# mym-br/gama_tts

Measured on AMD Instinct MI355X. Metric: audio samples/sec (whole node), batched VTM @44.1kHz, higher is better.
Workload: dtype f32

## Files before the change

### gama_tts_amd/capi.py

```python
import ctypes
import os

import numpy as np

_HERE = os.path.dirname(os.path.abspath(__file__))
_LIB_NAME = "libgama_vtm.so"
N_PARAM = 16
DEVICE_NONE = -1
PRECISION_F64 = 0
PRECISION_MIXED = 1
PRECISION_F32 = 2
TUBE_10_6 = 0
TUBE_30_18 = 1
TABLE_FIR, TABLE_SRC_H, TABLE_SRC_DH, TABLE_WAVETABLE = 0, 1, 2, 3
_STATUS_UNSUPPORTED = 4


class GvtmError(RuntimeError):
    def __init__(self, status, message):
        super().__init__("gvtm status %d: %s" % (status, message))
        self.status = status


class Config(ctypes.Structure):
# ... 132 lines not shown
        "gvtm_tracks_frame_count": (sz, [tracks, vp, sz]),
        "gvtm_generate_tracks_device": (i, [i, tracks, vp, vp, sz, sz, vp, vp, vp, vp]),
        "gvtm_synthesize_events_device": (i, [vp, tracks, vp, vp, sz, sz, vp, sz, vp, vp, vp, vp, vp]),
        "gvtm_plan_set_voice_tracks": (i, [vp, tracks, sz]),
        "gvtm_generate_tracks_voices_device": (i, [vp, vp, vp, vp, sz, sz, vp, vp, vp, vp]),
        "gvtm_synthesize_events_voices_device": (i, [vp, vp, vp, vp, sz, sz, vp, sz, vp, vp, vp, vp, vp]),
        "gvtm_tracks_chunks_frame_count": (sz, [tracks, vp, vp, sz]),
        "gvtm_generate_tracks_chunks_device": (i, [vp, vp, vp, vp, vp, sz, sz, vp, vp, vp, vp]),
        "gvtm_synthesize_events_chunks_device": (i, [vp, vp, vp, vp, vp, sz, sz, vp, sz, vp, vp, vp, vp, vp]),
        "gvtm_intonation_apply_host": (i64, [tracks, vp, sz, vp, sz, vp, sz, vp]),
        "gvtm_apply_intonation_device": (i, [vp, vp, vp, sz, vp, vp, vp, vp, sz, vp, sz, vp, vp, vp]),
        "gvtm_synthesize_intonation_device": (i, [vp, vp, vp, sz, vp, vp, vp, vp, sz, sz, sz, vp, sz, vp, vp, vp, vp, vp, vp]),
        "gvtm_modification_filter_length": (i64, [vp, i]),
        "gvtm_modification_apply_host": (i, [vp, i, vp, sz, vp, vp, sz, vp, vp, vp, vp]),
        "gvtm_apply_modifications_device": (i, [vp, vp, vp, sz, vp, vp, vp, vp, vp, vp, vp, sz, sz, vp, vp, vp, vp]),
        "gvtm_synthesize_modified_device": (i, [vp, vp, vp, sz, vp, vp, vp, vp, vp, vp, vp, sz, sz, vp, sz, vp, vp, vp, vp, vp]),
        "gvtm_stream_push_events": (i, [vp, vp, vp, vp, vp, sz, vp, vp]),
        "gvtm_stream_get_drift": (i, [vp, vp]),
        "gvtm_stream_set_drift": (i, [vp, vp]),
        "gvtm_events_packed_layout": (sz, [vp, vp, vp, vp, vp, sz, vp, vp]),
        "gvtm_synthesize_events_packed_host": (i, [vp, vp, vp, vp, vp, sz, vp, sz, vp, vp, vp, sz, vp, vp, vp]),
        "gvtm_synthesize_events_packed_host_pcm16": (i, [vp, vp, vp, vp, vp, sz, vp, sz, vp, vp, vp, sz, vp, vp, vp, vp]),
        "gvtm_generate_tracks_host": (i, [i, tracks, vp, vp, sz, sz, vp, vp, vp]),
    }
    hooks = {
        "gvtm_debug_set_rows": (i, [vp, i]),
        "gvtm_debug_lds_bytes": (sz, [vp, i]),
        "gvtm_debug_launch_shape": (i, [vp, sz, i, vp]),
        "gvtm_debug_stream_launch_shape": (i, [vp, sz, vp]),
        "gvtm_debug_chunk_length": (i, [vp, sz]),
        "gvtm_debug_fir_literals": (i, [vp]),
        "gvtm_debug_plan_fir_literals": (i, [vp]),
        "gvtm_debug_force_generic_fir": (i, [vp]),
        "gvtm_debug_noise_table": (i, [sz, i, vp]),
        "gvtm_debug_set_taps": (i, [vp, vp]),
        "gvtm_debug_set_phase_cycles": (i, [vp, vp]),
        "gvtm_debug_dpp_selftest": (i, [vp, vp]),
        "gvtm_debug_short_math": (i, [i, vp, sz, vp]),
        "gvtm_debug_device_float_math": (i, [vp, i, vp, sz, vp]),
        "gvtm_debug_group_voices": (i, [vp, vp, sz, i, vp, vp, vp, vp]),
        "gvtm_debug_tracks_append": (i, [vp, vp, vp, vp, vp, vp, sz, sz, vp, vp, vp]),
        "gvtm_debug_tracks_slice": (i, [vp, vp, i64, vp, vp, vp, vp, sz, sz, vp, vp, vp, vp]),
        "gvtm_debug_carry_rows": (i, [vp, vp, vp, vp, sz, sz]),
    }
    return product, hooks


PROTOTYPES, HOOK_PROTOTYPES = _prototypes()
_REQUIRED = (
    "gvtm_status_string", "gvtm_last_error", "gvtm_device_count", "gvtm_plan_create", "gvtm_plan_create_model5", "gvtm_plan_destroy",
    "gvtm_plan_info", "gvtm_plan_table", "gvtm_output_count", "gvtm_output_capacity", "gvtm_synthesize_batch_device",
    "gvtm_synthesize_batch_host", "gvtm_synthesize_batch_host_pcm16", "gvtm_host_alloc", "gvtm_host_free", "gvtm_normalize_batch_device",
    "gvtm_tracks_frame_count", "gvtm_generate_tracks_device", "gvtm_synthesize_events_device", "gvtm_generate_tracks_host",
    "gvtm_stream_create", "gvtm_stream_destroy", "gvtm_stream_reset", "gvtm_stream_capacity", "gvtm_stream_push", "gvtm_stream_finish",
    "gvtm_plan_set_timing", "gvtm_plan_take_kernel_ms")


def library_path(diagnostics=False):
    return os.path.join(_HERE, "lib", "libgama_vtm_diag.so" if diagnostics else _LIB_NAME)


_libs = {}


def load_library(diagnostics=False):
    if diagnostics in _libs:
# ... 260 lines not shown
                raise ValueError("rows can only be forced on a diagnostics plan")
            self._check(self._lib.gvtm_debug_set_rows(self._h, int(rows)))

    def _check(self, rc):
        if rc != 0:
            _check(self._lib, rc)

    def close(self):
        if self._h:
            self._lib.gvtm_plan_destroy(self._h)
            self._h = ctypes.c_void_p()

    def __del__(self):
        try:
            self.close()
        except Exception:
            pass

    def table(self, which):
        buf = np.empty(4096, dtype=np.float64)
        n = self._lib.gvtm_plan_table(self._h, which, buf.ctypes.data, buf.size)
        if n < 0:
            self._check(-n)
        return buf[:n].copy()

    def uses_fir_literals(self):
        rc = self._lib.gvtm_debug_plan_fir_literals(self._h)
        if rc < 0:
            self._check(-rc)
        return bool(rc)

    def force_generic_fir(self):
        self._check(self._lib.gvtm_debug_force_generic_fir(self._h))

    def output_count(self, frames):
        return int(self._lib.gvtm_output_count(self._h, int(frames)))

    def output_capacity(self, max_frames):
        return int(self._lib.gvtm_output_capacity(self._h, int(max_frames)))

    def set_timing(self, enabled):
        self._check(self._lib.gvtm_plan_set_timing(self._h, int(bool(enabled))))

    def take_kernel_ms(self):
        n = ctypes.c_int(0)
        ms = self._lib.gvtm_plan_take_kernel_ms(self._h, ctypes.byref(n))
        return float(ms), int(n.value)

    def synthesize_device(self, d_params, batch, max_frames, d_audio, audio_stride, d_frame_counts=None,
                          d_out_counts=None, d_maxabs=None, stream=None):
        self._check(self._lib.gvtm_synthesize_batch_device(
            self._h, _ptr(d_params), _ptr(d_frame_counts), int(batch), int(max_frames), _ptr(d_audio),
            int(audio_stride), _ptr(d_out_counts), _ptr(d_maxabs), _ptr(stream)))

    @staticmethod
    def _host_outputs(batch, shape, dtype):
        return (np.zeros(shape, dtype=dtype), np.zeros(batch, dtype=np.int64), np.zeros(batch, dtype=np.float32),
                np.zeros(batch, dtype=np.float32) if dtype == np.int16 else None)

    def _host(self, params, frame_counts, dtype):
        params = np.ascontiguousarray(params, dtype=np.float32)
        assert params.ndim == 3 and params.shape[2] == N_PARAM
        batch, frames = params.shape[:2]
        assert frame_counts is None or np.shape(frame_counts) == (batch,)
        stride = self.output_count(frames) if frame_counts is None else self.output_capacity(frames)
        out, counts, maxabs, scales = self._host_outputs(batch, (batch, stride), dtype)
# ... 359 lines not shown
```

### gama_tts_amd/csrc/vtm_capi_hooks.cpp

```cpp
#include <cstring>

#include "vtm_host.hpp"
#include "vtm_math.hpp"

using namespace gvtm::host;

static int finish_kernel(hipError_t launched, const char* what)
{
	const hipError_t e = launched == hipSuccess ? hipDeviceSynchronize() : launched;
	return e == hipSuccess ? GVTM_OK : fail_hip(e, what);
}

extern "C" {

#pragma GCC visibility push(default)

int gvtm_debug_set_rows(gvtm_plan* plan, int rows)
{
	if (!plan) return fail(GVTM_ERR_INVALID_ARGUMENT, "null plan");
	plan->rows = rows;
	return GVTM_OK;
}

size_t gvtm_debug_lds_bytes(const gvtm_plan* plan, int rows)
// ... 17 lines not shown
	if (plan->designs[0].model5) return fail(GVTM_ERR_UNSUPPORTED, "a plan of the models 0 to 4");
	const gvtm::LaunchShape shape = plan->stream_launch_shape(batch, 0, plan->longest_stream_ring());
	if (!shape.rows) return fail(GVTM_ERR_UNSUPPORTED, "LDS budget exceeded");
	out[0] = static_cast<size_t>(shape.rows), out[1] = static_cast<size_t>(shape.ring), out[2] = shape.lds;
	return GVTM_OK;
}

int gvtm_debug_chunk_length(const gvtm_plan* plan, size_t batch)
{
	if (!plan) return -fail(GVTM_ERR_INVALID_ARGUMENT, "null plan");
	if (plan->designs[0].model5) return 0;
	const gvtm::LaunchShape shape = plan->launch_shape(batch, 0, false);
	if (!shape.rows) return 0;
	return gvtm::synth_chunk_length(plan->designs[0].k, plan->precision, shape.rows);
}

int gvtm_debug_fir_literals(float* out)
{
	if (!out) return fail(GVTM_ERR_INVALID_ARGUMENT, "null buffer");
	std::memcpy(out, gvtm::kGlottalFirF32, sizeof(gvtm::kGlottalFirF32));
	return gvtm::kGlottalFirTapsF32;
}

int gvtm_debug_plan_fir_literals(const gvtm_plan* plan)
{
	if (!plan) return -fail(GVTM_ERR_INVALID_ARGUMENT, "null plan");
	return plan->fir_literals ? 1 : 0;
}

int gvtm_debug_force_generic_fir(gvtm_plan* plan)
{
	if (!plan) return fail(GVTM_ERR_INVALID_ARGUMENT, "null plan");
	plan->fir_literals = false;
	return GVTM_OK;
}

int gvtm_debug_noise_table(size_t n, int as_float, void* out)
{
	if (!out) return fail(GVTM_ERR_INVALID_ARGUMENT, "null buffer");
	gvtm::design_noise_table(n, as_float != 0, out);
	return GVTM_OK;
}

int gvtm_debug_set_taps(gvtm_plan* plan, double* d_taps)
{
	if (!plan) return fail(GVTM_ERR_INVALID_ARGUMENT, "null plan");
	plan->debug_taps = d_taps;
	return GVTM_OK;
}

int gvtm_debug_set_phase_cycles(gvtm_plan* plan, unsigned long long* d_cycles)
{
	if (!plan) return fail(GVTM_ERR_INVALID_ARGUMENT, "null plan");
	plan->phase_cycles = d_cycles;
	return GVTM_OK;
}

int gvtm_debug_dpp_selftest(gvtm_plan* plan, int* out)
{
	if (!plan || !out || plan->device == GVTM_DEVICE_NONE) return fail(GVTM_ERR_INVALID_ARGUMENT, "needs a device plan");
	DeviceScope scope(plan->device);
	if (const int rc = scope.entered(); rc != GVTM_OK) return rc;
	DeviceBuffer d;
	hipError_t e = d.ensure(gvtm::kDppSelftestInts * sizeof(int));
	if (e == hipSuccess) e = gvtm::launch_dpp_selftest(d.as<int>(), nullptr);
	if (e != hipSuccess) return fail_hip(e, "dpp selftest");
// ... 104 lines not shown
```

### gama_tts_amd/csrc/vtm_capi_launch.cpp

```cpp
#include <cstring>

#include "vtm_host.hpp"

#ifndef GVTM_NOISE_TABLE
#define GVTM_NOISE_TABLE 1
#endif

using namespace gvtm::host;

namespace {

int use_noise_table(gvtm_plan* plan, size_t steps, gvtm::SynthArgs& args)
{
	constexpr size_t kNoiseTableMaxSteps = size_t(1) << 26;
	if (steps > kNoiseTableMaxSteps) {
	} else if (steps > plan->noise_len) {
		size_t want = ((steps + (size_t(1) << 18) - 1) >> 18) << 18;
		want = std::min(std::max(want, 2 * plan->noise_len), kNoiseTableMaxSteps);
		std::vector<unsigned char> host(want * sizeof(float));
		gvtm::design_noise_table(want, true, host.data());
		DeviceBuffer fresh;
		if (const int rc = upload(fresh, host, "upload noise table"); rc != GVTM_OK) return rc;
		if (plan->d_noise.ptr) plan->noise_retired.push_back(std::move(plan->d_noise));
		plan->d_noise = std::move(fresh);
		plan->noise_len = want;
	}
	if (steps <= kNoiseTableMaxSteps) {
		args.noise_lp = plan->d_noise.ptr;
		args.noise_len = plan->noise_len;
	}
	return GVTM_OK;
}

gvtm::SynthArgs synth_args(const gvtm_plan* plan, const LaunchRequest& r)
{
	const gvtm::Design& dg = plan->designs[0];
	gvtm::SynthArgs args;
	args.k = dg.k;
	args.kconst = static_cast<const gvtm::DeviceConstants*>(plan->d_consts.ptr);
	args.params = r.params;
	args.frame_counts = r.frame_counts;
	args.audio = r.audio;
	args.out_counts = r.out_counts;
	args.maxabs = r.maxabs;
	args.wavetable = plan->d_wavetable.ptr;
	args.fir = plan->d_fir.ptr;
	std::memset(&args.fir_k, 0, sizeof(args.fir_k));
	args.fir_literals = plan->fir_literals ? 1 : 0;
	if (!dg.model5) {
		if (dg.f32) {
			for (size_t i = 0; i < dg.fir_f.size() && i < static_cast<size_t>(gvtm::kFirKConsts); ++i) args.fir_k.f[i] = dg.fir_f[i];
			float* kf = args.fir_k.f + gvtm::kFirKConsts;
			for (int q = 0; q < 8; ++q) kf[gvtm::kKfRadiusCoef + q] = static_cast<float>(dg.k.radius_coef[q]);
			kf[gvtm::kKfAperture2] = static_cast<float>(dg.k.aperture_radius2);
			kf[gvtm::kKfNasalR2Sq] = static_cast<float>(dg.k.nasal_r2_sq);
			kf[gvtm::kKfBasicIncrement] = static_cast<float>(dg.k.basic_increment);
			kf[gvtm::kKfBpT] = static_cast<float>(dg.k.bp_T);
			kf[gvtm::kKfBreathiness] = static_cast<float>(dg.k.breathiness);
			kf[gvtm::kKfCrossmix] = static_cast<float>(dg.k.crossmix_factor);
			kf[gvtm::kKfThroatB0] = static_cast<float>(dg.k.throat_b0);
			kf[gvtm::kKfThroatA1] = static_cast<float>(dg.k.throat_a1);
			kf[gvtm::kKfThroatGain] = static_cast<float>(dg.k.throat_gain);
			kf[gvtm::kKfMouthARad] = static_cast<float>(dg.k.mouth_a_rad);
			kf[gvtm::kKfNoseARad] = static_cast<float>(dg.k.nose_a_rad);
			kf[gvtm::kKfNasalK5] = static_cast<float>(dg.k.nasal_k[5]);
		}
	}
	args.src_h = plan->d_src_h.ptr;
	args.src_dh = plan->d_src_dh.ptr;
	args.max_frames = r.max_frames;
	args.audio_stride = r.audio_stride;
	args.batch = r.batch;
	if (r.sl) {
		args.stream = r.sl->d_state;
		args.stream_stride = r.sl->stride;
		args.stream_mode = r.sl->mode;
		if (r.voices && !dg.model5) args.stream_chunk = gvtm::synth_chunk_length(dg.k, plan->precision, 1);
	}
	args.debug_taps = r.voices ? nullptr : plan->debug_taps;
	args.phase_cycles = r.voices ? nullptr : plan->phase_cycles;
	args.k5const = static_cast<const gvtm::Model5Constants*>(plan->d_consts5.ptr);
// ... 153 lines not shown
```

### gama_tts_amd/csrc/vtm_capi_plan.cpp

```cpp
#include <cstring>
#include <memory>
#include <new>

#include "vtm_host.hpp"

namespace gvtm::host {

thread_local std::string g_last_error;

int fail(int status, const std::string& msg)
{
	g_last_error = msg;
	return status;
}

int fail_hip(hipError_t e, const char* what)
{
	return fail(GVTM_ERR_HIP, std::string(what) + ": " + hipGetErrorString(e));
}

int check_device_index(int device, const char* what)
{
	int n = 0;
	if (hipGetDeviceCount(&n) != hipSuccess || n <= 0) return fail(GVTM_ERR_NO_DEVICE, std::string("no HIP device available (") + what + " has no CPU path)");
// ... 14 lines not shown
	hipDeviceProp_t prop;
	if (const hipError_t e = hipGetDeviceProperties(&prop, device); e != hipSuccess) return fail_hip(e, "hipGetDeviceProperties");
	if (std::strncmp(prop.gcnArchName, "gfx950", 6) != 0) {
		return fail(GVTM_ERR_NO_DEVICE, std::string("kernels are built for gfx950 only, device is ") + prop.gcnArchName);
	}
	plan->compute_units = prop.multiProcessorCount;
	return GVTM_OK;
}

int upload_tables(gvtm_plan* plan)
{
	const gvtm::Design& dg = plan->designs[0];
	std::vector<gvtm::DeviceConstants> consts;
	std::vector<gvtm::Model5Constants> consts5;
	std::vector<double> wavetables;
	std::vector<float> wavetables_f;
	for (const gvtm::Design& dv : plan->designs) {
		consts.push_back(dv.k);
		if (dg.model5) consts5.push_back(dv.k5);
		wavetables.insert(wavetables.end(), dv.wavetable.begin(), dv.wavetable.end());
		wavetables_f.insert(wavetables_f.end(), dv.wavetable_f.begin(), dv.wavetable_f.end());
	}
	auto upload_design = [&](DeviceBuffer& dst, const std::vector<double>& wide, const std::vector<float>& narrow, const char* what) {
		return dg.f32 ? upload(dst, narrow, what) : upload(dst, wide, what);
	};
	int rc = GVTM_OK;
	if (!dg.model5) {
		if ((rc = upload_design(plan->d_wavetable, wavetables, wavetables_f, "upload wavetable")) != GVTM_OK) return rc;
		if ((rc = upload_design(plan->d_fir, dg.fir, dg.fir_f, "upload fir")) != GVTM_OK) return rc;
	}
	if ((rc = upload_design(plan->d_src_h, dg.src_h, dg.src_h_f, "upload src_h")) != GVTM_OK) return rc;
	if ((rc = upload_design(plan->d_src_dh, dg.src_dh, dg.src_dh_f, "upload src_dh")) != GVTM_OK) return rc;
	if ((rc = upload(plan->d_consts, consts, "upload constants")) != GVTM_OK) return rc;
	return dg.model5 ? upload(plan->d_consts5, consts5, "upload model 5 constants") : GVTM_OK;
}

template <typename Config, typename Differs>
int create_plan(const Config* configs, size_t n_voices, double control_rate, int device, gvtm_plan** plan_out, const char* shared_keys,
		Differs differs, std::string (*design)(const Config&, double, gvtm::Design&), bool float5_voices = false)
{
	if (!configs || !plan_out) return fail(GVTM_ERR_INVALID_ARGUMENT, "null config or plan_out");
	*plan_out = nullptr;
	if (n_voices == 0) return fail(GVTM_ERR_INVALID_ARGUMENT, "a plan needs at least one voice");
	if (n_voices > 0x7fffffffu) return fail(GVTM_ERR_INVALID_ARGUMENT, "too many voices");
	for (size_t v = 1; v < n_voices; ++v) {
		if (differs(configs[0], configs[v])) {
			return fail(GVTM_ERR_INVALID_ARGUMENT, "voice " + std::to_string(v) + ": " + shared_keys + " must be those of voice 0 "
					"(one plan is one model at one output rate)");
		}
	}
	try {
		std::unique_ptr<gvtm_plan, void (*)(gvtm_plan*)> plan(new gvtm_plan, gvtm_plan_destroy);
		plan->designs.resize(n_voices);
		for (size_t v = 0; v < n_voices; ++v) {
			const std::string why = design(configs[v], control_rate, plan->designs[v]);
			if (!why.empty()) return fail(GVTM_ERR_INVALID_ARGUMENT, n_voices > 1 ? "voice " + std::to_string(v) + ": " + why : why);
		}
		plan->precision = configs[0].precision;
		plan->float5_voices = float5_voices;
		const gvtm::Design& d0 = plan->designs[0];
		plan->fir_literals = !d0.model5 && d0.f32 && d0.fir_f.size() == static_cast<size_t>(gvtm::kGlottalFirTapsF32)
				&& std::memcmp(d0.fir_f.data(), gvtm::kGlottalFirF32, sizeof(gvtm::kGlottalFirF32)) == 0;
		if (device == GVTM_DEVICE_NONE) {
			plan->device = GVTM_DEVICE_NONE;
			*plan_out = plan.release();
			return GVTM_OK;
		}
		int rc = open_device(plan.get(), device);
		if (rc != GVTM_OK) return rc;
		DeviceScope scope(device);
		if ((rc = scope.entered()) != GVTM_OK || (rc = upload_tables(plan.get())) != GVTM_OK) return rc;
		*plan_out = plan.release();
		return GVTM_OK;
	} catch (const std::bad_alloc&) {
		return fail(GVTM_ERR_OUT_OF_MEMORY, "host allocation failed");
	} catch (const std::exception& ex) {
		return fail(GVTM_ERR_INVALID_ARGUMENT, ex.what());
	}
}

void fill_info(const gvtm_plan* plan, const gvtm::Design& dg, gvtm_info* info)
{
	const gvtm::DeviceConstants& k = dg.k;
	info->internal_sample_rate = k.sample_rate;
	info->control_steps = k.control_steps;
	info->output_rate = dg.config.output_rate;
	info->control_rate = dg.control_rate;
	info->fir_taps = k.fir_taps;
	info->time_register_increment = k.time_inc;
	info->phase_increment = k.phase_inc;
	info->pad_size = k.pad;
	info->upsampling = k.upsampling;
	info->device = plan->device;
	info->precision = plan->precision;
	info->section_delay = k.section_delay;
// ... 242 lines not shown
```

### gama_tts_amd/csrc/vtm_design.cpp

```cpp
#include "vtm_design.hpp"
#include "vtm_intonation.hpp"

#include <algorithm>
#include <cmath>
#include <sstream>

namespace gvtm {

namespace {

constexpr double kPi = 3.14159265358979323846;


struct Rational { int numerator, denominator, order; };

template <typename T>
Rational best_rational(T value, int order)
{
	constexpr int kLimit = 200;
	Rational r{0, 0, -1};
	if (order <= 0) return r;
	const T frac = std::abs(value - static_cast<int>(value));
	const int max_den = std::min(2 * order, kLimit);
	T best = 1.0;
// ... 261 lines not shown
	if (c.tube_layout == GVTM_TUBE_30_18 && c.section_delay != 1) return "the 30+18-section tube (VocalTractModel4) runs with section_delay 1";
	if (c.precision != GVTM_PRECISION_F64 && c.precision != GVTM_PRECISION_MIXED && c.precision != GVTM_PRECISION_F32) return "unknown precision";
	if (!(c.glottal_pulse_tp > 0.0) || c.glottal_pulse_tn_min < 0.0 || c.glottal_pulse_tn_max < c.glottal_pulse_tn_min ||
			c.glottal_pulse_tp + c.glottal_pulse_tn_max > 100.0) {
		return "glottal pulse shape needs tp > 0, 0 <= tn_min <= tn_max, tp + tn_max <= 100";
	}
	if (!(c.temperature > -273.0) || !std::isfinite(c.temperature)) return "temperature out of range";

	out.config = c;
	out.control_rate = control_rate;
	DeviceConstants& k = out.k;
	k = DeviceConstants{};
	k.section_delay = c.section_delay;
	k.layout = c.tube_layout;
	k.waveform = c.waveform;
	k.modulation = c.noise_modulation != 0;
	out.f32 = c.precision == GVTM_PRECISION_F32;
	if (out.f32) {
		Tables<float> tb;
		const std::string msg = design_numbers<float>(c, control_rate, k, tb);
		if (!msg.empty()) return msg;
		out.fir_f = tb.fir; out.src_h_f = tb.src_h; out.src_dh_f = tb.src_dh; out.wavetable_f = tb.wavetable;
		out.fir.assign(tb.fir.begin(), tb.fir.end());
		out.src_h.assign(tb.src_h.begin(), tb.src_h.end());
		out.src_dh.assign(tb.src_dh.begin(), tb.src_dh.end());
		out.wavetable.assign(tb.wavetable.begin(), tb.wavetable.end());
		return "";
	}
	Tables<double> tb;
	const std::string msg = design_numbers<double>(c, control_rate, k, tb);
	if (!msg.empty()) return msg;
	out.fir = tb.fir; out.src_h = tb.src_h; out.src_dh = tb.src_dh; out.wavetable = tb.wavetable;
	return "";
}

void design_noise_table(size_t n, bool as_float, void* out)
{
	double seed = 0.7892347;
	if (as_float) {
		float* o = static_cast<float*>(out);
		float prev = 0.0f;
		for (size_t i = 0; i < n; ++i) {
			const double product = seed * 377.0;
			seed = product - std::floor(product);
			const float white = static_cast<float>(seed - 0.5);
			o[i] = white + prev;
			prev = white;
		}
	} else {
		double* o = static_cast<double*>(out);
		double prev = 0.0;
		for (size_t i = 0; i < n; ++i) {
			const double product = seed * 377.0;
			seed = product - std::floor(product);
			const double white = seed - 0.5;
			o[i] = white + prev;
			prev = white;
		}
	}
}

namespace {

template <typename T>
void radiation_impedance_t(T radius, T period, double out[6])
{
// ... 286 lines not shown
```

### gama_tts_amd/csrc/vtm_design.hpp

```cpp
#pragma once

#include <cstddef>
#include <cstdint>
#include <string>
#include <vector>

#include "../../include/gama_vtm.h"

namespace gvtm {

constexpr int kWavetableLength = 512;
constexpr int kSrcZeroCrossings = 13;
constexpr int kSrcPhases = 256;
constexpr int kSrcFilterLength = kSrcZeroCrossings * kSrcPhases;
constexpr int kSrcRing = 1024;
constexpr int kMaxFirTaps = 64;
constexpr int kMaxSectionDelay = 4;
constexpr int kMaxPad = 96;

constexpr int kGlottalFirTapsF32 = 47;
constexpr float kGlottalFirF32[kGlottalFirTapsF32] = {
	0x1.7104f6p-24f, 0x1.e9efcap-23f, -0x1.a0e112p-25f, -0x1.45ce18p-19f,
	-0x1.a55396p-18f, 0x1.2af00ap-19f, 0x1.6ac7fap-15f, 0x1.246622p-14f,
	-0x1.6c9652p-14f, -0x1.c5647cp-12f, -0x1.2c53bp-12f, 0x1.28a494p-10f,
// ... 42 lines not shown
	double sample_rate;
	double output_rate;
	int bypass, constant_mouth;
	double rb_t1, rb_tn_min, rb_tn_max;
	double gn_b0, gn_a1;
	double gp_b0, gp_a1;
	double fn_b0, fn_b1, fn_a1, fn_a2;
	double frication_factor;
	double min_loss, max_loss;
	double nasal_r1_sq;
	double nasal_k[6];
	double period;
	double nose_c[6];
	double mouth_c[6];
};

struct Design {
	bool model5 = false;
	gvtm5_config config5{};
	Model5Constants k5{};
	gvtm_config config;
	double control_rate;
	DeviceConstants k;
	std::vector<double> fir;
	std::vector<double> src_h;
	std::vector<double> src_dh;
	std::vector<double> wavetable;
	bool f32 = false;
	std::vector<float> fir_f, src_h_f, src_dh_f, wavetable_f;
};

void design_noise_table(size_t n, bool as_float, void* out);

std::string design_plan(const gvtm_config& cfg, double control_rate, Design& out);

std::string design_plan5(const gvtm5_config& cfg, double control_rate, Design& out);
std::string design_plan5_float(const gvtm5_config& cfg, double control_rate, Design& out);

void radiation_impedance(double radius, double period, double out[6]);

double amplitude_60db(double db);

#if defined(__HIPCC__)
#define GVTM_DESIGN_HD __host__ __device__ inline
#else
#define GVTM_DESIGN_HD inline
#endif

GVTM_DESIGN_HD int synth_ring_for(int upsampling, int pad, int chunk)
{
	if (!upsampling) return kSrcRing;
	int xr = 128;
	while (xr < 2 * chunk + 4 * pad + 64) xr *= 2;
	return xr;
}

GVTM_DESIGN_HD bool src_flush_overrun(unsigned time_inc, int pad, uint64_t steps, uint64_t& k_from, uint64_t& k_to)
{
	const uint64_t fills = steps + 2ull * static_cast<uint64_t>(pad);
	const uint64_t fill_size = static_cast<uint64_t>(kSrcRing - 2 * pad);
	const uint64_t last_auto_end = (fills / fill_size) * fill_size;
	k_from = ((fills << 16) + time_inc - 1) / time_inc;
	k_to = k_from;
	if (last_auto_end == 0) return false;
	const uint64_t k_star = ((last_auto_end << 16) + time_inc - 1) / time_inc;
	const uint64_t p_star = (k_star * static_cast<uint64_t>(time_inc)) >> 16;
// ... 61 lines not shown
```

### gama_tts_amd/csrc/vtm_host.hpp

```cpp
#pragma once
#include <hip/hip_runtime.h>

#include <algorithm>
#include <cstdint>
#include <string>
#include <utility>
#include <vector>

#include "../../include/gama_vtm.h"
#include "vtm_design.hpp"
#include "vtm_kernels.hpp"
#include "vtm_tracks.hpp"

namespace gvtm::host {

int fail(int status, const std::string& msg);
int fail_hip(hipError_t e, const char* what);

struct DeviceBuffer {
	void* ptr = nullptr;
	size_t bytes = 0;
	DeviceBuffer() = default;
	DeviceBuffer(DeviceBuffer&& o) noexcept : ptr(std::exchange(o.ptr, nullptr)), bytes(std::exchange(o.bytes, 0)) {}
	DeviceBuffer& operator=(DeviceBuffer&& o) noexcept
// ... 40 lines not shown
};

class DeviceScope {
public:
	explicit DeviceScope(int device)
	{
		if (hipGetDevice(&previous_) != hipSuccess) previous_ = -1;
		status_ = (previous_ == device) ? hipSuccess : hipSetDevice(device);
		changed_ = status_ == hipSuccess && previous_ != device;
	}
	~DeviceScope()
	{
		if (changed_ && previous_ >= 0) (void) hipSetDevice(previous_);
	}
	DeviceScope(const DeviceScope&) = delete;
	DeviceScope& operator=(const DeviceScope&) = delete;
	int entered() const { return status_ == hipSuccess ? GVTM_OK : fail_hip(status_, "hipSetDevice"); }
private:
	int previous_ = -1;
	bool changed_ = false;
	hipError_t status_ = hipSuccess;
};

}

struct gvtm_plan {
	using DeviceBuffer = gvtm::host::DeviceBuffer;
	std::vector<gvtm::Design> designs;
	int device = 0;
	int precision = GVTM_PRECISION_F64;
	int rows = 0;
	bool float5_voices = false;
	bool fir_literals = false;
	DeviceBuffer d_wavetable, d_fir, d_src_h, d_src_dh;
	DeviceBuffer d_consts, d_consts5;
	DeviceBuffer d_noise;
	size_t noise_len = 0;
	std::vector<DeviceBuffer> noise_retired;
	struct {
		DeviceBuffer frames, voice_ids, counts, maxabs, scales, groups;
		DeviceBuffer params, audio, pcm;
		DeviceBuffer set[3], frame_offsets, sample_offsets;
		DeviceBuffer chunk_offsets, utt_chunks, drift;
		size_t limit = 0;
		size_t slices = 0, largest_slice = 0;
		size_t staging_bytes() const { return set[0].bytes + set[1].bytes + set[2].bytes; }
		void release_sets() { for (DeviceBuffer& s : set) s = DeviceBuffer(); }
		unsigned char* set_of(size_t i) const { return set[i % 3].as<unsigned char>(); }
	} host;
	struct {
		DeviceBuffer params, frames, groups;
		DeviceBuffer events, event_offsets;
	} async;
	std::vector<gvtm::TrackConstants> voice_tracks;
	DeviceBuffer d_voice_tracks;
	int compute_units = 0;
	bool timing = false;
	double* debug_taps = nullptr;
	unsigned long long* phase_cycles = nullptr;
	std::vector<gvtm::host::EventPair> pending, pool;
	gvtm::host::Stream h2d_stream, compute_stream, copy_stream;
	std::vector<gvtm::host::Event> slice_events;

	int n_voices() const { return static_cast<int>(designs.size()); }
	gvtm::LaunchShape launch_shape(size_t batch, int forced_rows, bool voices, int stream_ring = 0, bool fit = true) const
	{
// ... 189 lines not shown
```

### gama_tts_amd/csrc/vtm_kernel_v2.inc

```

namespace v2 {

namespace {

constexpr int kPrm = 17;
constexpr int kF1Planes = 6;
constexpr int kF1U = 0, kF1Sig = 1, kF1Thr = 2, kF1B0 = 3, kF1A1 = 4, kF1A2 = 5;
constexpr int kKl = 11;
constexpr int kKlK8 = 7, kKlNk1 = 8, kKlAlr = 9, kKlAu = 10;
constexpr int kInj = 9;
template <typename CT, int LAYOUT>
constexpr bool lane_rec()
{
	return sizeof(CT) == 4 && LAYOUT == 0;
}
constexpr int kLrZero = 16, kLrAlr = 17, kLrAu = 18, kLrK8 = 19, kLrKn = 20, kLrInj = 21, kLrLen = 31;
constexpr int kl_len(bool lr)
{
	return lr ? kLrLen : kKl;
}
template <typename CT>
constexpr bool fr_compact()
{
	return sizeof(CT) == 8;
// ... 11 lines not shown
}
template <int C, int U>
constexpr int rec_slot(int rec)
{
	return U * C * rec + rec_pad<C>(rec) * ((U + 1) / 2);
}
template <int C, int U>
__host__ __device__ constexpr size_t rec_at(int rec, int slot, int u)
{
	return static_cast<size_t>(slot) * rec_slot<C, U>(rec) + static_cast<size_t>(u) * (C * rec) + static_cast<size_t>(rec_pad<C>(rec)) * ((u + 1) / 2);
}
constexpr int kDump = 64 * 4;
constexpr int kXMirror = 32;
constexpr int kWPre = 48;
static_assert(kWPre == kStreamPreRoll, "a stream state carries one pre-roll");

struct Extent {
	int frames;
	int nchunks;
	uint32_t steps;
	int last_frame;
	unsigned long long step_base;
	unsigned long long k_first;
};

#ifndef GVTM_KERNEL_TAPS
#define GVTM_KERNEL_TAPS 0
#endif
#ifndef GVTM_TUNE_SKIP
#define GVTM_TUNE_SKIP 0
#endif
#ifndef GVTM_TUNE_TRACE
#define GVTM_TUNE_TRACE 0
#endif
constexpr unsigned kSerialHelpMask = 0x1a;
template <typename CT, typename ST, int U>
constexpr bool kSrcHOnly = sizeof(ST) == 8 && U > 1;
template <typename CT, typename ST, int U, int C>
struct Smem {
	DeviceConstants* kc;
	Extent* ext;
	CT* wavetable;
	CT* fir;
	SrcTap<ST>* src;
	float* prm;
	CT* inc;
	CT* amp;
	CT* pos;
	CT* noise;
	CT* w;
	CT* usg;
	CT* fr;
	CT* kl;
	CT* inj;
	CT* lanec;
	CT* thy;
	CT* ox;
	CT* opk;
	ST* x;
	unsigned* peak;
	unsigned long long* kb;
	unsigned* ticket;
	unsigned long long* diag;
	CT* dump;
};

// ... 142 lines not shown
			{kCopy, -1, 3, 1, -1},
			c,
			{kJunction, -1, 0, 0, -1},
			{kCopy, -1, 4, 1, -1},
			c,
			{kJunction, -1, 0, 0, -1},
			{kCopy, -1, 5, 1, -1},
			c,
			{kEnd, -1, 0, 0, -1},
		};
		return t[L < 48 ? L : 47];
	}
};

}

template <int U, int LAYOUT>
constexpr int serial_waves()
{
	return TubeLayout<LAYOUT>::kWaveWide ? U + 4 : 5 * ((U + 3) / 4);
}

constexpr int kVoicesFlag = 2;

__device__ __forceinline__ size_t voice_row(const SynthArgs& a, size_t slot)
{
	const int r = a.row_map[slot];
	return r < 0 ? a.batch : static_cast<size_t>(r);
}

template <int D, int U> constexpr bool far_calls_inline() { return D == 1 && U == 4; }
template <int D, int U> constexpr bool fir_literal_taps() { return !((D == 1 && U == 1) || (D == 2 && U == 2)); }
template <typename CT, int D, int U, int LAYOUT> constexpr bool bounds_by_recurrence() { return sizeof(CT) == 4 && U == 4 && LAYOUT == 0 && (D == 2 || D == 3); }
template <typename CT, int D, int U, bool VOICES> constexpr bool float_arg_consts() { return sizeof(CT) == 4 && !VOICES && !far_calls_inline<D, U>(); }

template <typename CT, typename ST, int D, int U, int C, int NH, int LAYOUT_FLAGS>
__global__ __launch_bounds__((serial_waves<U, LAYOUT_FLAGS & 1>() + NH) * 64) void vtm_synth_kernel(const SynthArgs a)
{
	constexpr int LAYOUT = LAYOUT_FLAGS & 1;
	constexpr bool VOICES = (LAYOUT_FLAGS & kVoicesFlag) != 0;
	int voice = 0;
	if constexpr (VOICES) {
		voice = a.group_voice[blockIdx.x];
		if (voice < 0) return;
	}
	using TL = TubeLayout<LAYOUT>;
	static_assert(!TL::kWaveWide || U <= 4, "wave-wide tubes: one tube wavefront per utterance, at most four");
	constexpr int kSerial = serial_waves<U, LAYOUT>();
	static_assert(C % D == 0, "chunk must be a multiple of the section delay");
	static_assert(U == 1 || U == 2 || U == 4 || U == 8, "utterances per workgroup = DPP rows used");
	constexpr int G = (U + 3) / 4;
	static_assert(2 * C >= kWPre, "FIR pre-roll copy needs 2C >= kWPre");
	const int XR = VOICES ? synth_ring_for(a.kconst[voice].upsampling, a.kconst[voice].pad, a.stream ? a.stream_chunk : C) : a.xr;
	const int XRS = XR + kXMirror;
	static_assert(NH >= 1, "at least one helper wavefront");
	constexpr int kThreads = (kSerial + NH) * 64;

	extern __shared__ __attribute__((aligned(16))) unsigned char smem_raw[];
	constexpr bool kLaneRec = lane_rec<CT, LAYOUT>();
	constexpr SmemOffsets<CT, ST, U, C, kLaneRec> so;
	Smem<CT, ST, U, C> sm;
	sm.kc = reinterpret_cast<DeviceConstants*>(smem_raw + so.kc);
	sm.ext = reinterpret_cast<Extent*>(smem_raw + so.ext);
	sm.wavetable = reinterpret_cast<CT*>(smem_raw + so.wavetable);
	sm.fir = reinterpret_cast<CT*>(smem_raw + so.fir);
	sm.src = reinterpret_cast<SrcTap<ST>*>(smem_raw + so.src);
// ... 7 lines not shown
	sm.fr = reinterpret_cast<CT*>(smem_raw + so.fr);
	sm.kl = reinterpret_cast<CT*>(smem_raw + so.kl);
	sm.inj = reinterpret_cast<CT*>(smem_raw + so.inj);
	sm.lanec = reinterpret_cast<CT*>(smem_raw + so.lanec);
	sm.thy = reinterpret_cast<CT*>(smem_raw + so.thy);
	sm.ox = reinterpret_cast<CT*>(smem_raw + so.ox);
	sm.opk = reinterpret_cast<CT*>(smem_raw + so.opk);
	sm.x = reinterpret_cast<ST*>(smem_raw + so.x);
	sm.peak = reinterpret_cast<unsigned*>(smem_raw + so.peak);
	sm.dump = reinterpret_cast<CT*>(smem_raw + so.dump);
	sm.diag = reinterpret_cast<unsigned long long*>(smem_raw + so.diag);
	sm.ticket = reinterpret_cast<unsigned*>(smem_raw + so.ticket);
	sm.kb = reinterpret_cast<unsigned long long*>(smem_raw + so.kb);

	const int tid = threadIdx.x;
	const int lane = tid & 63;
	const int wave = tid >> 6;
	const int hl = lane;
	const size_t group = blockIdx.x;
#define GVTM_ROW_UTT(u, ...) (VOICES ? voice_row(a, group * U + (u)) : __VA_ARGS__)
	constexpr bool kArgConsts = float_arg_consts<CT, D, U, VOICES>();
	constexpr bool kFarInline = far_calls_inline<D, U>();
#define GVTM_KF(idx, field) (kArgConsts ? static_cast<CT>(a.fir_k.f[kFirKConsts + (idx)]) : CT(k.field))
	constexpr int kFr = fr_len<CT>();
	constexpr bool kFrCompact = fr_compact<CT>();
	auto at_prm = [](int slot, int u) { return rec_at<C, U>(kPrm, slot, u); };
	auto at_usg = [](int slot, int u) { return rec_at<C, U>(kF1Planes, slot, u); };
	auto at_fr = [](int slot, int u) { return rec_at<C, U>(fr_len<CT>(), slot, u); };
	constexpr bool kMaskedSerial = sizeof(ST) == 4;
	constexpr int kStaticRounds = (U == 4 && LAYOUT == 0 && (sizeof(CT) == 4 || (sizeof(ST) == 8 ? D <= 2 : D == 1))) ? 1 : 0;
	constexpr bool kHelperByRole = sizeof(CT) == 4 || D >= 3 || (sizeof(ST) == 8 && D == 2);
	constexpr bool kNoiseTable = sizeof(CT) == 4;
	constexpr bool kBoundsRecurrence = bounds_by_recurrence<CT, D, U, LAYOUT>();
	constexpr int kKlLen = kl_len(kLaneRec);
	constexpr int kInjLen = kLaneRec ? kKlLen : kInj;
	auto at_kl = [](int slot, int u) { return rec_at<C, U>(kKlLen, slot, u); };
	constexpr bool kBlockRec = kLaneRec && D != 3;
	auto kl_index = [](int s, int e) -> int {
		if constexpr (kBlockRec) return (s >> 2) * (kKlLen * 4) + e * 4 + (s & 3);
		else return s * kKlLen + e;
	};
	auto at_inj = [](int slot, int u) { return kLaneRec ? rec_at<C, U>(kKlLen, slot, u) + kLrInj : rec_at<C, U>(kInj, slot, u); };
	auto amp_at = [](int slot, int u, int which, int s) -> size_t {
		return ((static_cast<size_t>(slot) * U + u) * 2 + which) * C + s;
	};
	const bool kPush = a.stream_mode == kStreamPush;
	const bool kFinal = !kPush;
	using SL = StreamLayout<CT, ST>;
	constexpr int kTubeLanes = TubeLayout<LAYOUT>::kLanes;
	constexpr int kTubeWords = 2 * D + 1;

	{
		const int* src = reinterpret_cast<const int*>(VOICES ? a.kconst + voice : a.kconst);
		int* dst = reinterpret_cast<int*>(sm.kc);
		for (int i = tid; i < static_cast<int>(sizeof(DeviceConstants) / sizeof(int)); i += kThreads) dst[i] = src[i];
	}
	for (int i = tid; i < kWavetableLength; i += kThreads) sm.wavetable[i] = VOICES ? static_cast<const CT*>(a.wavetable)[static_cast<size_t>(voice) * kWavetableLength + i] : static_cast<const CT*>(a.wavetable)[i];
	for (int i = tid; i < kSrcFilterLength; i += kThreads) {
		if constexpr (kSrcHOnly<CT, ST, U>) {
			reinterpret_cast<ST*>(sm.src)[i] = static_cast<ST>(static_cast<const CT*>(a.src_h)[i]);
			if (i == 0) reinterpret_cast<ST*>(sm.src)[kSrcFilterLength] = ST(0);
		} else {
			sm.src[i].h = static_cast<ST>(static_cast<const CT*>(a.src_h)[i]);
			sm.src[i].dh = static_cast<ST>(static_cast<const CT*>(a.src_dh)[i]);
		}
	}
// ... 162 lines not shown
				for (int i = 0; i < kTubeWords; ++i) st[i] = tb[i];
			}
		}
	}

	unsigned long long role_busy = 0;
#if GVTM_TUNE_TRACE
	int tr_n = 0;
	auto TR = [&](int t, unsigned id) {
		if (a.phase_cycles != nullptr && group == 0 && lane == 0 && t >= GVTM_TUNE_TRACE && t < GVTM_TUNE_TRACE + 2 && tr_n < 128)
			a.phase_cycles[32768 + wave * 128 + tr_n++] = (static_cast<unsigned long long>(id) << 48) | (clock64() & 0xFFFFFFFFFFFFull);
	};
#else
	auto TR = [](int, unsigned) {};
#endif
	const bool stamping = a.phase_cycles != nullptr && lane == 0;


	auto stage_p2a = [&](int c, int pass) {
		for (int item = pass * 64 + hl; item < U * C && item < (pass + 1) * 64; item += 64) {
			const int u = item / C, s = item - u * C;
			if (s >= valid_in(u, c)) continue;
			const float* pv = sm.prm + at_prm(c & 1, u) + s * kPrm;
			const CT pitch = pv[0], gv = pv[1], av = pv[2];
			const CT f0 = frequency_dev<kFarInline>(pitch);
			sm.inc[((c & 1) * U + u) * C + s] = (f0 / CT(2.0)) * GVTM_KF(kKfBasicIncrement, basic_increment);
			sm.amp[amp_at(c & 3, u, 0, s)] = amplitude_60db_dev<kFarInline>(gv);
			sm.amp[amp_at(c & 3, u, 1, s)] = amplitude_60db_dev<kFarInline>(av);
		}
	};

	constexpr int kP4aItems = 1;
	auto stage_p4a = [&](int c, int pass) {
		if constexpr (U == 1) {
			for (int item = pass * 64 + hl; item < U * 2 * C && item < (pass + 1) * 64; item += 64) {
				const int u = item / (2 * C), h = item - u * 2 * C;
				if (h >= 2 * valid_in(u, c)) continue;
				const CT p = sm.pos[((c & 1) * U + u) * 2 * C + h];
				const unsigned lower = static_cast<unsigned>(static_cast<int>(p));
				const unsigned upper = (lower + 1 > 511u) ? lower + 1 - 512u : lower + 1;
				const CT ax = sm.amp[amp_at(c & 3, u, 0, h >> 1)];
				const CT wl = wavetable_entry(sm.wavetable, k, lower, ax);
				const CT wu = wavetable_entry(sm.wavetable, k, upper, ax);
				const CT v = wl + rmul(p - static_cast<CT>(lower), wu - wl);
				CT* slot = sm.w + (static_cast<size_t>(c % 3) * U + u) * (kWPre + 2 * C);
				slot[kWPre + h] = v;
				if (GVTM_KERNEL_TAPS && a.debug_taps) {
					a.debug_taps[(GVTM_ROW_UTT(u, (group * U + u)) * a.max_frames * k.control_steps + static_cast<size_t>(c) * C + (h >> 1)) * 8 + 5 + (h & 1)] = p;
				}
				if (h >= 2 * C - kWPre) {
					CT* next = sm.w + (static_cast<size_t>((c + 1) % 3) * U + u) * (kWPre + 2 * C);
					next[h - (2 * C - kWPre)] = v;
				}
			}
			return;
		}
		int item[kP4aItems], u[kP4aItems], h[kP4aItems];
		bool on[kP4aItems];
		CT p[kP4aItems], ax[kP4aItems];
#pragma unroll
		for (int q = 0; q < kP4aItems; ++q) {
			item[q] = (pass * kP4aItems + q) * 64 + hl;
			u[q] = item[q] / (2 * C);
			h[q] = item[q] - u[q] * 2 * C;
			on[q] = item[q] < U * 2 * C && h[q] < 2 * valid_in(u[q] < U ? u[q] : 0, c);
			if (!on[q]) { u[q] = 0; h[q] = 0; }
// ... 261 lines not shown
#pragma unroll
				for (int u = 0; u < UG; ++u) acc[u] = mad(xs[u], coef, acc[u]);
			}
		};
		auto tap = [&](int ri, ST coef) {
			ST xs[UG];
#pragma unroll
			for (int u = 0; u < UG; ++u) xs[u] = xg[u * XRS + ri];
			tapv(xs, coef);
		};
		if (k.upsampling) {
			const unsigned l = frac >> 8, m = frac & 0xFFu;
			const ST interp = static_cast<ST>(m) / ST(256);
			const int lo = (base - (kSrcZeroCrossings - 1)) & (XR - 1);
			const unsigned nfrac = (~frac) & 0xFFFFu;
			const unsigned l2 = nfrac >> 8, m2 = nfrac & 0xFFu;
			const ST interp2 = static_cast<ST>(m2) / ST(256);
			if constexpr (sizeof(CT) == 4) {
			auto wing = [&](unsigned lbase, ST ip, int x0, int xstep) {
				constexpr int kZ = kSrcZeroCrossings;
				SrcTap<ST> cf[kZ];
				ST xv[kZ][UG];
#pragma unroll
				for (int j = 0; j < kZ; ++j) cf[j] = src_tap(lbase + 256 * j);
#pragma unroll
				for (int j = 0; j < kZ; ++j) {
#pragma unroll
					for (int u = 0; u < UG; ++u) xv[j][u] = xg[u * XRS + x0 + xstep * j];
				}
				asm volatile("" ::: "memory");
#pragma unroll
				for (int j = 0; j < kZ; ++j) tapv(xv[j], mad(cf[j].dh, ip, cf[j].h));
			};
			wing(l, interp, lo + (kSrcZeroCrossings - 1), -1);
			wing(l2, interp2, lo + kSrcZeroCrossings, 1);
			} else if constexpr (U >= 4) {
				constexpr int kG = 4;
				auto wing_groups = [&](unsigned lbase, ST ip, int x0, int xstep) {
#pragma unroll
					for (int j0 = 0; j0 < kSrcZeroCrossings; j0 += kG) {
						SrcTap<ST> cf[kG];
						ST xv[kG][UG];
#pragma unroll
						for (int g = 0; g < kG; ++g) {
							if (j0 + g < kSrcZeroCrossings) {
								cf[g] = src_tap(lbase + 256 * (j0 + g));
#pragma unroll
								for (int u = 0; u < UG; ++u) xv[g][u] = xg[u * XRS + x0 + xstep * (j0 + g)];
							}
						}
						asm volatile("" ::: "memory");
#pragma unroll
						for (int g = 0; g < kG; ++g) {
							if (j0 + g < kSrcZeroCrossings) tapv(xv[g], mad(cf[g].dh, ip, cf[g].h));
						}
					}
				};
				wing_groups(l, interp, lo + (kSrcZeroCrossings - 1), -1);
				wing_groups(l2, interp2, lo + kSrcZeroCrossings, 1);
			} else {
#pragma unroll
			for (int j = 0; j < kSrcZeroCrossings; ++j) {
				const SrcTap<ST> cf = src_tap(l + 256 * j);
				const ST coef = mad(cf.dh, interp, cf.h);
				tap(lo + (kSrcZeroCrossings - 1 - j), coef);
			}
#pragma unroll
			for (int j = 0; j < kSrcZeroCrossings; ++j) {
// ... 832 lines not shown
```

### gama_tts_amd/csrc/vtm_kernels.hpp

```cpp
#pragma once

#include <hip/hip_runtime.h>

#include <cstddef>
#include <cstdint>

#include "vtm_design.hpp"

namespace gvtm {

struct StreamHeader {
	unsigned long long step_base;
	double seed;
	unsigned peak_bits;
	unsigned reserved_;
	unsigned long long pad_;
};
static_assert(sizeof(StreamHeader) == 32, "stream header layout");
constexpr int kStreamScalars = 12;
constexpr int kSsPos = 0, kSsPrev = 1;
constexpr int kSsBp = 2, kSsThr = 6;
constexpr int kSsRadMouth = 7, kSsRadNose = 9;
constexpr int kStreamPreRoll = 48;
enum StreamMode : int { kStreamNone = 0, kStreamPush = 1, kStreamFinish = 2 };
// ... 30 lines not shown
};
constexpr int kFirKConsts = 64;

struct SynthArgs {
	DeviceConstants k;
	const DeviceConstants* kconst;
	const float* params;
	const int32_t* frame_counts;
	float* audio;
	int64_t* out_counts;
	float* maxabs;
	const void* wavetable;
	const void* fir;
	union FirByValue { double d[49]; float f[98]; } fir_k;
	static_assert(sizeof(FirByValue) == sizeof(double) * 49 && kFirKConsts + kKfCount <= 98, "float constants fit behind the float coefficients");
	const void* src_h;
	const void* src_dh;
	const void* noise_lp = nullptr;
	unsigned long long noise_len = 0;
	size_t max_frames;
	size_t audio_stride;
	size_t batch;
	int xr;
	unsigned char* stream = nullptr;
	size_t stream_stride = 0;
	int stream_mode = kStreamNone;
	double* debug_taps;
	unsigned long long* phase_cycles;
	const Model5Constants* k5const = nullptr;
	const int32_t* row_map = nullptr;
	const int32_t* group_voice = nullptr;
	int stream_chunk = 0;
	int fir_literals = 0;
};

struct GroupVoicesArgs {
	const int32_t* voice_ids;
	size_t batch;
	int n_voices;
	int rows;
	size_t groups;
	int32_t* row_map;
	int32_t* group_voice;
	int32_t* counts;
	int64_t* out_counts;
	float* maxabs;
};
constexpr int kGroupVoicesThreads = 256;

struct NormalizeArgs {
	const float* audio;
	const int64_t* counts;
	const float* maxabs;
	float* out_f32;
	int16_t* out_i16;
	float* scales;
	size_t audio_stride;
};

struct LaunchShape {
	int rows = 0;
	int ring = 0;
	size_t lds = 0;
	int forced = 0;
	int per_cu = 0;
};
// ... 19 lines not shown
```

Before: 17.04 billion.

## Add precomputed sample-rate-converter phase table and static wavetable fast path

Precomputes per-phase interpolated resampler filter coefficients on the host when the time increment yields a small periodic set of phases, uploads them, and lets the f32 single-voice kernel load whole 16-byte coefficient records instead of doing the table interpolation per output sample. It also adds a simplified wavetable lookup pass for configurations where the glottal wavetable does not change. Both are gated by plan flags and compile-time shape predicates, with debug hooks to force the generic paths. The cost is extra global memory traffic for the phase table and more kernel code and register pressure.

```diff
diff --git a/gama_tts_amd/capi.py b/gama_tts_amd/capi.py
--- a/gama_tts_amd/capi.py
+++ b/gama_tts_amd/capi.py
@@ -188,6 +188,11 @@
         "gvtm_debug_fir_literals": (i, [vp]),
         "gvtm_debug_plan_fir_literals": (i, [vp]),
         "gvtm_debug_force_generic_fir": (i, [vp]),
+        "gvtm_debug_plan_src_phases": (i, [vp]),
+        "gvtm_debug_plan_src_phase_table": (i, [vp, vp, sz]),
+        "gvtm_debug_force_generic_src": (i, [vp]),
+        "gvtm_debug_plan_static_wavetable": (i, [vp]),
+        "gvtm_debug_force_dynamic_wavetable": (i, [vp]),
         "gvtm_debug_noise_table": (i, [sz, i, vp]),
         "gvtm_debug_set_taps": (i, [vp, vp]),
         "gvtm_debug_set_phase_cycles": (i, [vp, vp]),
@@ -514,6 +519,31 @@
 
     def force_generic_fir(self):
         self._check(self._lib.gvtm_debug_force_generic_fir(self._h))
+
+    def _hook_count(self, rc):
+        if rc < 0:
+            self._check(-rc)
+        return int(rc)
+
+    def src_phases(self):
+        return self._hook_count(self._lib.gvtm_debug_plan_src_phases(self._h))
+
+    def src_phase_table(self):
+        phases = self.src_phases()
+        if not phases:
+            return None
+        out = np.empty((phases, 28), dtype=np.float32)
+        assert self._hook_count(self._lib.gvtm_debug_plan_src_phase_table(self._h, out.ctypes.data, out.size)) == phases
+        return out
+
+    def force_generic_src(self):
+        self._check(self._lib.gvtm_debug_force_generic_src(self._h))
+
+    def says_static_wavetable(self):
+        return bool(self._hook_count(self._lib.gvtm_debug_plan_static_wavetable(self._h)))
+
+    def force_dynamic_wavetable(self):
+        self._check(self._lib.gvtm_debug_force_dynamic_wavetable(self._h))
 
     def output_count(self, frames):
         return int(self._lib.gvtm_output_count(self._h, int(frames)))
diff --git a/gama_tts_amd/csrc/vtm_capi_hooks.cpp b/gama_tts_amd/csrc/vtm_capi_hooks.cpp
--- a/gama_tts_amd/csrc/vtm_capi_hooks.cpp
+++ b/gama_tts_amd/csrc/vtm_capi_hooks.cpp
@@ -73,6 +73,42 @@
 {
 	if (!plan) return fail(GVTM_ERR_INVALID_ARGUMENT, "null plan");
 	plan->fir_literals = false;
+	return GVTM_OK;
+}
+
+int gvtm_debug_plan_src_phases(const gvtm_plan* plan)
+{
+	if (!plan) return -fail(GVTM_ERR_INVALID_ARGUMENT, "null plan");
+	return static_cast<int>(plan->src_phases);
+}
+
+int gvtm_debug_plan_src_phase_table(const gvtm_plan* plan, float* out, size_t capacity)
+{
+	if (!plan || !out) return -fail(GVTM_ERR_INVALID_ARGUMENT, "null plan or buffer");
+	if (!plan->src_phases) return 0;
+	const std::vector<float> table = gvtm::design_src_phase_table(plan->designs[0]);
+	if (capacity < table.size()) return -fail(GVTM_ERR_INVALID_ARGUMENT, "table buffer too small");
+	std::memcpy(out, table.data(), sizeof(float) * table.size());
+	return static_cast<int>(plan->src_phases);
+}
+
+int gvtm_debug_force_generic_src(gvtm_plan* plan)
+{
+	if (!plan) return fail(GVTM_ERR_INVALID_ARGUMENT, "null plan");
+	plan->src_phases = 0;
+	return GVTM_OK;
+}
+
+int gvtm_debug_plan_static_wavetable(const gvtm_plan* plan)
+{
+	if (!plan) return -fail(GVTM_ERR_INVALID_ARGUMENT, "null plan");
+	return plan->static_wavetable ? 1 : 0;
+}
+
+int gvtm_debug_force_dynamic_wavetable(gvtm_plan* plan)
+{
+	if (!plan) return fail(GVTM_ERR_INVALID_ARGUMENT, "null plan");
+	plan->static_wavetable = false;
 	return GVTM_OK;
 }
 
diff --git a/gama_tts_amd/csrc/vtm_capi_launch.cpp b/gama_tts_amd/csrc/vtm_capi_launch.cpp
--- a/gama_tts_amd/csrc/vtm_capi_launch.cpp
+++ b/gama_tts_amd/csrc/vtm_capi_launch.cpp
@@ -47,6 +47,11 @@
 	args.fir = plan->d_fir.ptr;
 	std::memset(&args.fir_k, 0, sizeof(args.fir_k));
 	args.fir_literals = plan->fir_literals ? 1 : 0;
+	if (plan->src_phases) {
+		args.src_phase = plan->d_src_phase.as<float>();
+		args.src_phase_mask = plan->src_phases - 1;
+	}
+	args.static_wavetable = plan->static_wavetable ? 1 : 0;
 	if (!dg.model5) {
 		if (dg.f32) {
 			for (size_t i = 0; i < dg.fir_f.size() && i < static_cast<size_t>(gvtm::kFirKConsts); ++i) args.fir_k.f[i] = dg.fir_f[i];
diff --git a/gama_tts_amd/csrc/vtm_capi_plan.cpp b/gama_tts_amd/csrc/vtm_capi_plan.cpp
--- a/gama_tts_amd/csrc/vtm_capi_plan.cpp
+++ b/gama_tts_amd/csrc/vtm_capi_plan.cpp
@@ -70,6 +70,15 @@
 	if ((rc = upload_design(plan->d_src_h, dg.src_h, dg.src_h_f, "upload src_h")) != GVTM_OK) return rc;
 	if ((rc = upload_design(plan->d_src_dh, dg.src_dh, dg.src_dh_f, "upload src_dh")) != GVTM_OK) return rc;
 	if ((rc = upload(plan->d_consts, consts, "upload constants")) != GVTM_OK) return rc;
+	if (plan->src_phases) {
+		const std::vector<float> table = gvtm::design_src_phase_table(dg);
+		if (plan->d_src_phase.ensure(sizeof(float) * table.size()) != hipSuccess) {
+			(void) hipGetLastError();
+			plan->src_phases = 0;
+		} else if (const hipError_t e = hipMemcpy(plan->d_src_phase.ptr, table.data(), sizeof(float) * table.size(), hipMemcpyHostToDevice); e != hipSuccess) {
+			return fail_hip(e, "upload converter phase table");
+		}
+	}
 	return dg.model5 ? upload(plan->d_consts5, consts5, "upload model 5 constants") : GVTM_OK;
 }
 
@@ -99,6 +108,10 @@
 		const gvtm::Design& d0 = plan->designs[0];
 		plan->fir_literals = !d0.model5 && d0.f32 && d0.fir_f.size() == static_cast<size_t>(gvtm::kGlottalFirTapsF32)
 				&& std::memcmp(d0.fir_f.data(), gvtm::kGlottalFirF32, sizeof(gvtm::kGlottalFirF32)) == 0;
+		if (n_voices == 1 && !d0.model5) {
+			plan->src_phases = gvtm::src_phase_count(d0);
+			plan->static_wavetable = gvtm::static_wavetable(d0.k);
+		}
 		if (device == GVTM_DEVICE_NONE) {
 			plan->device = GVTM_DEVICE_NONE;
 			*plan_out = plan.release();
diff --git a/gama_tts_amd/csrc/vtm_design.cpp b/gama_tts_amd/csrc/vtm_design.cpp
--- a/gama_tts_amd/csrc/vtm_design.cpp
+++ b/gama_tts_amd/csrc/vtm_design.cpp
@@ -317,6 +317,35 @@
 	if (!msg.empty()) return msg;
 	out.fir = tb.fir; out.src_h = tb.src_h; out.src_dh = tb.src_dh; out.wavetable = tb.wavetable;
 	return "";
+}
+
+unsigned src_phase_count(const Design& d)
+{
+	const DeviceConstants& k = d.k;
+	if (d.model5 || !d.f32 || !k.upsampling || k.time_inc == 0 || k.time_inc > 65536u) return 0;
+	const unsigned low_bit = k.time_inc & (0u - k.time_inc);
+	const unsigned phases = 65536u / low_bit;
+	return phases <= kSrcPhaseCap ? phases : 0;
+}
+
+std::vector<float> design_src_phase_table(const Design& d)
+{
+	const unsigned phases = src_phase_count(d);
+	std::vector<float> table(static_cast<size_t>(phases) * kSrcPhaseRecord, 0.0f);
+	for (unsigned p = 0; p < phases; ++p) {
+		float* rec = table.data() + static_cast<size_t>(p) * kSrcPhaseRecord;
+		const unsigned frac = (p * d.k.time_inc) & 0xFFFFu;
+		const unsigned wing_frac[2] = {frac, (~frac) & 0xFFFFu};
+		for (int w = 0; w < 2; ++w) {
+			const unsigned l = wing_frac[w] >> 8;
+			const float interp = static_cast<float>(wing_frac[w] & 0xFFu) / 256.0f;
+			for (int j = 0; j < kSrcZeroCrossings; ++j) {
+				const float product = d.src_dh_f[l + 256 * j] * interp;
+				rec[w * kSrcZeroCrossings + j] = d.src_h_f[l + 256 * j] + product;
+			}
+		}
+	}
+	return table;
 }
 
 void design_noise_table(size_t n, bool as_float, void* out)
diff --git a/gama_tts_amd/csrc/vtm_design.hpp b/gama_tts_amd/csrc/vtm_design.hpp
--- a/gama_tts_amd/csrc/vtm_design.hpp
+++ b/gama_tts_amd/csrc/vtm_design.hpp
@@ -98,6 +98,12 @@
 
 void design_noise_table(size_t n, bool as_float, void* out);
 
+constexpr int kSrcPhaseRecord = 28;
+constexpr unsigned kSrcPhaseCap = 16384;
+unsigned src_phase_count(const Design& d);
+std::vector<float> design_src_phase_table(const Design& d);
+inline bool static_wavetable(const DeviceConstants& k) { return k.tn_delta == 0.0 || k.waveform != 0; }
+
 std::string design_plan(const gvtm_config& cfg, double control_rate, Design& out);
 
 std::string design_plan5(const gvtm5_config& cfg, double control_rate, Design& out);
diff --git a/gama_tts_amd/csrc/vtm_host.hpp b/gama_tts_amd/csrc/vtm_host.hpp
--- a/gama_tts_amd/csrc/vtm_host.hpp
+++ b/gama_tts_amd/csrc/vtm_host.hpp
@@ -96,6 +96,9 @@
 	int rows = 0;
 	bool float5_voices = false;
 	bool fir_literals = false;
+	unsigned src_phases = 0;
+	DeviceBuffer d_src_phase;
+	bool static_wavetable = false;
 	DeviceBuffer d_wavetable, d_fir, d_src_h, d_src_dh;
 	DeviceBuffer d_consts, d_consts5;
 	DeviceBuffer d_noise;
diff --git a/gama_tts_amd/csrc/vtm_kernel_v2.inc b/gama_tts_amd/csrc/vtm_kernel_v2.inc
--- a/gama_tts_amd/csrc/vtm_kernel_v2.inc
+++ b/gama_tts_amd/csrc/vtm_kernel_v2.inc
@@ -67,6 +67,9 @@
 #endif
 #ifndef GVTM_TUNE_TRACE
 #define GVTM_TUNE_TRACE 0
+#endif
+#ifndef GVTM_TUNE_PLAN_TABLES
+#define GVTM_TUNE_PLAN_TABLES (-1)
 #endif
 constexpr unsigned kSerialHelpMask = 0x1a;
 template <typename CT, typename ST, int U>
@@ -275,6 +278,18 @@
 template <int D, int U> constexpr bool far_calls_inline() { return D == 1 && U == 4; }
 template <int D, int U> constexpr bool fir_literal_taps() { return !((D == 1 && U == 1) || (D == 2 && U == 2)); }
 template <typename CT, int D, int U, int LAYOUT> constexpr bool bounds_by_recurrence() { return sizeof(CT) == 4 && U == 4 && LAYOUT == 0 && (D == 2 || D == 3); }
+template <typename CT, int D, int U, int LAYOUT, bool VOICES> constexpr bool src_phase_table()
+{
+	constexpr bool can = sizeof(CT) == 4 && !VOICES;
+	if (GVTM_TUNE_PLAN_TABLES >= 0) return can && (GVTM_TUNE_PLAN_TABLES & 1) != 0;
+	return can && LAYOUT == 0 && ((U == 4 && D == 1) || (U == 2 && D == 2));
+}
+template <typename CT, int D, int U, int LAYOUT, bool VOICES> constexpr bool static_wavetable_pass()
+{
+	constexpr bool can = sizeof(CT) == 4 && !VOICES;
+	if (GVTM_TUNE_PLAN_TABLES >= 0) return can && (GVTM_TUNE_PLAN_TABLES & 2) != 0;
+	return can && LAYOUT == 0 && ((U == 4 && (D == 1 || D == 2)) || (U == 2 && D == 2));
+}
 template <typename CT, int D, int U, bool VOICES> constexpr bool float_arg_consts() { return sizeof(CT) == 4 && !VOICES && !far_calls_inline<D, U>(); }
 
 template <typename CT, typename ST, int D, int U, int C, int NH, int LAYOUT_FLAGS>
@@ -348,6 +363,8 @@
 	constexpr bool kHelperByRole = sizeof(CT) == 4 || D >= 3 || (sizeof(ST) == 8 && D == 2);
 	constexpr bool kNoiseTable = sizeof(CT) == 4;
 	constexpr bool kBoundsRecurrence = bounds_by_recurrence<CT, D, U, LAYOUT>();
+	constexpr bool kSrcPhaseTable = src_phase_table<CT, D, U, LAYOUT, VOICES>();
+	constexpr bool kStaticWavetablePass = static_wavetable_pass<CT, D, U, LAYOUT, VOICES>();
 	constexpr int kKlLen = kl_len(kLaneRec);
 	constexpr int kInjLen = kLaneRec ? kKlLen : kInj;
 	auto at_kl = [](int slot, int u) { return rec_at<C, U>(kKlLen, slot, u); };
@@ -576,6 +593,30 @@
 
 	constexpr int kP4aItems = 1;
 	auto stage_p4a = [&](int c, int pass) {
+		if constexpr (kStaticWavetablePass) {
+			if (a.static_wavetable != 0) {
+				static_assert(kP4aItems == 1, "one item per lane and pass");
+				const int item = pass * 64 + hl;
+				const int u = item / (2 * C), h = item - u * 2 * C;
+				if (item >= U * 2 * C || h >= 2 * valid_in(u, c)) return;
+				const CT p = sm.pos[((c & 1) * U + u) * 2 * C + h];
+				const unsigned lower = static_cast<unsigned>(static_cast<int>(p));
+				const unsigned upper = (lower + 1 > 511u) ? lower + 1 - 512u : lower + 1;
+				const CT wl = sm.wavetable[lower];
+				const CT wu = sm.wavetable[upper];
+				const CT v = wl + rmul(p - static_cast<CT>(lower), wu - wl);
+				CT* slot = sm.w + (static_cast<size_t>(c % 3) * U + u) * (kWPre + 2 * C);
+				slot[kWPre + h] = v;
+				if (GVTM_KERNEL_TAPS && a.debug_taps) {
+					a.debug_taps[(GVTM_ROW_UTT(u, (group * U + u)) * a.max_frames * k.control_steps + static_cast<size_t>(c) * C + (h >> 1)) * 8 + 5 + (h & 1)] = p;
+				}
+				if (h >= 2 * C - kWPre) {
+					CT* next = sm.w + (static_cast<size_t>((c + 1) % 3) * U + u) * (kWPre + 2 * C);
+					next[h - (2 * C - kWPre)] = v;
+				}
+				return;
+			}
+		}
 		if constexpr (U == 1) {
 			for (int item = pass * 64 + hl; item < U * 2 * C && item < (pass + 1) * 64; item += 64) {
 				const int u = item / (2 * C), h = item - u * 2 * C;
@@ -903,8 +944,36 @@
 #pragma unroll
 				for (int j = 0; j < kZ; ++j) tapv(xv[j], mad(cf[j].dh, ip, cf[j].h));
 			};
+			if constexpr (kSrcPhaseTable) {
+				if (a.src_phase != nullptr) {
+					using F4 = float __attribute__((ext_vector_type(4)));
+					constexpr int kZ = kSrcZeroCrossings;
+					static_assert(kSrcPhaseRecord % 4 == 0 && 2 * kZ <= kSrcPhaseRecord, "a record: both wings in whole 16-byte loads");
+					const F4* rec = reinterpret_cast<const F4*>(a.src_phase + static_cast<size_t>(static_cast<unsigned>(ko) & a.src_phase_mask) * kSrcPhaseRecord);
+					F4 cq[kSrcPhaseRecord / 4];
+#pragma unroll
+					for (int q = 0; q < kSrcPhaseRecord / 4; ++q) cq[q] = rec[q];
+					auto wing_samples = [&](int c0, int x0, int xstep) {
+						ST xv[kZ][UG];
+#pragma unroll
+						for (int j = 0; j < kZ; ++j) {
+#pragma unroll
+							for (int u = 0; u < UG; ++u) xv[j][u] = xg[u * XRS + x0 + xstep * j];
+						}
+						asm volatile("" ::: "memory");
+#pragma unroll
+						for (int j = 0; j < kZ; ++j) tapv(xv[j], static_cast<ST>(cq[(c0 + j) >> 2][(c0 + j) & 3]));
+					};
+					wing_samples(0, lo + (kZ - 1), -1);
+					wing_samples(kZ, lo + kZ, 1);
+				} else {
+					wing(l, interp, lo + (kSrcZeroCrossings - 1), -1);
+					wing(l2, interp2, lo + kSrcZeroCrossings, 1);
+				}
+			} else {
 			wing(l, interp, lo + (kSrcZeroCrossings - 1), -1);
 			wing(l2, interp2, lo + kSrcZeroCrossings, 1);
+			}
 			} else if constexpr (U >= 4) {
 				constexpr int kG = 4;
 				auto wing_groups = [&](unsigned lbase, ST ip, int x0, int xstep) {
diff --git a/gama_tts_amd/csrc/vtm_kernels.hpp b/gama_tts_amd/csrc/vtm_kernels.hpp
--- a/gama_tts_amd/csrc/vtm_kernels.hpp
+++ b/gama_tts_amd/csrc/vtm_kernels.hpp
@@ -86,6 +86,9 @@
 	const int32_t* group_voice = nullptr;
 	int stream_chunk = 0;
 	int fir_literals = 0;
+	const float* src_phase = nullptr;
+	unsigned src_phase_mask = 0;
+	int static_wavetable = 0;
 };
 
 struct GroupVoicesArgs {
```

After: 17.29 billion, median of 6. 1.01x the previous value.
